# lyndonchan/wsss-analysis

Hardware: AMD Instinct MI355X
Metric: images/sec CAM+CRF pseudo-labels, VOC2012 321x321 (higher is better)
Workload: dtype f16x3; 1 GPU; resnet50 CAM + dense-CRF (M=21, 10 mean-field iters), 321x321, batch 32 images (=64 samples) per GPU, image-sharded; batch_images=32, num_classes=20, parallelism=image-sharded x1, no collective, steps_per_rank=239

## Files before the change

### __graft_entry__.py

```python
import os
import subprocess
import sys

ROOT = os.path.dirname(os.path.abspath(__file__))
PKG_DIR = os.path.join(ROOT, "wsss-analysis_amd")
CSRC = os.path.join(PKG_DIR, "csrc")
LIB_OUT = os.path.join(PKG_DIR, "wsscam", "libwsscam.so")
ORACLE_DIR = os.path.join(ROOT, "oracle")
ORACLE_OUT = os.path.join(ORACLE_DIR, "_build", "libdensecrf_ref.so")

HIP_SOURCES = ["api.hip", "conv_igemm.hip", "misc_kernels.hip", "net.hip", "cam_tail.hip", "crf.hip", "irn_kernels.hip", "rw.hip", "hsn.hip", "input.hip", "ir_label.hip", "stem_pool.hip", "cam_head.hip", "conv_f32.hip", "dsrg.hip", "cue_seeds.hip", "seg_eval.hip", "deeplab.hip", "seg_chain.hip", "seg_loss.hip", "pool.hip", "seg_grad.hip", "seg_sgd.hip", "seg_dropout.hip", "irn_loss.hip", "irn_grad.hip", "irn_sgd.hip", "irn_batch.hip", "seg_batch.hip", "cls_head.hip", "cls_grad.hip", "cls_sgd.hip"]
EXTRA_FLAGS = {"crf.hip": ["-ffp-contract=off"], "input.hip": ["-ffp-contract=off"], "deeplab.hip": ["-ffp-contract=off"],
               "seg_chain.hip": ["-ffp-contract=off"],
               "seg_sgd.hip": ["-ffp-contract=off"],
               "seg_dropout.hip": ["-ffp-contract=off"],
               "irn_sgd.hip": ["-ffp-contract=off"],
               "irn_grad.hip": ["-ffp-contract=off"],
               "irn_batch.hip": ["-ffp-contract=off"],
               "cls_sgd.hip": ["-ffp-contract=off"],
               "seg_batch.hip": ["-ffp-contract=off"]}


def _newer(target, deps):
    if not os.path.exists(target):
        return False
    t = os.path.getmtime(target)
    return all(os.path.getmtime(d) <= t for d in deps)


def _run(cmd):
    r = subprocess.run(cmd, stdout=subprocess.PIPE, stderr=subprocess.STDOUT, text=True)
    if r.returncode != 0:
        raise RuntimeError("command failed: %s\n%s" % (" ".join(cmd), r.stdout))
    return r.stdout


def build_lib(force=False, verbose=False):
    hipcc = os.environ.get("HIPCC", "/opt/rocm/bin/hipcc")
    objdir = os.path.join(PKG_DIR, "build")
    os.makedirs(objdir, exist_ok=True)
    os.makedirs(os.path.dirname(LIB_OUT), exist_ok=True)
    headers = [os.path.join(CSRC, "common.h"), os.path.join(CSRC, "bilerp.h"), os.path.join(CSRC, "tf_resize.h"),
               os.path.join(ROOT, "include", "wsscam.h")]
    if not force and _newer(LIB_OUT, [os.path.join(CSRC, src) for src in HIP_SOURCES] + headers):
        return LIB_OUT
    objs = []
    procs = []
    for src in HIP_SOURCES:
        sp = os.path.join(CSRC, src)
        op = os.path.join(objdir, src.replace(".hip", ".o"))
        objs.append(op)
        if not force and _newer(op, [sp] + headers):
            continue
        cmd = [hipcc, "--offload-arch=gfx950", "-O3", "-std=c++17", "-fPIC", "-Wall", "-c", sp, "-o", op] + EXTRA_FLAGS.get(src, [])
        if verbose:
            print(" ".join(cmd))
        procs.append((cmd, subprocess.Popen(cmd, stdout=subprocess.PIPE, stderr=subprocess.STDOUT, text=True)))
    for cmd, p in procs:
        out, _ = p.communicate()
        if p.returncode != 0:
            raise RuntimeError("hipcc failed: %s\n%s" % (" ".join(cmd), out))
        if verbose and out.strip():
            print(out)
    if force or procs or not _newer(LIB_OUT, objs):
        _run([hipcc, "--offload-arch=gfx950", "-shared", "-fPIC", "-o", LIB_OUT] + objs)
# ... 36 lines not shown
```

### include/wsscam.h

```cpp
#ifndef WSSCAM_H
#define WSSCAM_H

#include <stddef.h>
#include <stdint.h>

#ifdef __cplusplus
extern "C" {
#endif

#define WSC_VERSION 100

typedef enum wsc_status {
    WSC_OK = 0,
    WSC_ERR_INVALID = -1,
    WSC_ERR_NO_DEVICE = -2,
    WSC_ERR_HIP = -3,
    WSC_ERR_MISSING_KEY = -4,
    WSC_ERR_SHAPE = -5,
    WSC_ERR_NOMEM = -6,
    WSC_ERR_KEY_RANGE = -7,
    WSC_ERR_CAPACITY = -8,
    WSC_ERR_RANGE = -9
} wsc_status;

// ... 9 lines not shown
} wsc_arch;

typedef enum wsc_precision {
    WSC_PREC_BF16 = 0,
    WSC_PREC_BF16X3 = 1,
    WSC_PREC_F16 = 2,
    WSC_PREC_F16X3 = 3,
    WSC_PREC_F32 = 4
} wsc_precision;

typedef struct wsc_ctx wsc_ctx;
typedef struct wsc_net wsc_net;
typedef enum {
    WSC_OPT_CRF_GAUSS_ON_CHIP = 0,
    WSC_OPT_CRF_FUSED_BLUR = 1,
    WSC_OPT_CRF_BLUR_ON_CHIP = 2,
    WSC_OPT_CRF_RANK_BALLOT = 3,
    WSC_OPT_CRF_EMBED_FULL = 4,
    WSC_OPT_RW_TILED = 5,
    WSC_OPT_STEM_POOL_FUSED = 6,
    WSC_OPT_CONV_WINDOW = 7,
    WSC_OPT_CAM_HEAD_STREAM = 8,
    WSC_OPT_CRF_MSG_IN_UPDATE = 9,
    WSC_OPT_COUNT = 10
} wsc_option;

typedef struct wsc_crf wsc_crf;
typedef struct wsc_crf_v wsc_crf_v;

typedef struct wsc_tensor_desc {
    const char *name;
    const float *data;
    int32_t ndim;
    int64_t shape[4];
} wsc_tensor_desc;


int wsc_version(void);
const char *wsc_last_error(void);

int wsc_ctx_create(int device, void *stream, wsc_ctx **out);
void wsc_ctx_destroy(wsc_ctx *ctx);
int wsc_ctx_set_option(wsc_ctx *ctx, int option, int value);
int wsc_ctx_scratch_fill(wsc_ctx *ctx, int value);
int wsc_ctx_scratch_fill_value(const wsc_ctx *ctx);
int wsc_sync(wsc_ctx *ctx);
int wsc_ctx_range_status(wsc_ctx *ctx, int *flag_out, int clear);
// ... 401 lines not shown
```

### profiles/conv_layer_table.py

```python
import re
import sqlite3
import sys


def resnet50_layers(S):
    def o(h, k, s, p):
        return (h + 2 * p - k) // s + 1

    L = []
    h = o(S, 7, 2, 3)
    L.append(("stem 7x7 s2 3->64", h, 3, 64, 7))
    h = o(h, 3, 2, 1)
    inp = 64
    for li, (planes, blocks, stride) in enumerate(((64, 3, 1), (128, 4, 2), (256, 6, 2), (512, 3, 1)), 1):
        for b in range(blocks):
            s = stride if b == 0 else 1
            ho = o(h, 3, s, 1)
            n = "layer%d.%d." % (li, b)
            L.append((n + "conv1 1x1 %d->%d" % (inp, planes), h, inp, planes, 1))
            L.append((n + "conv2 3x3 %d s%d" % (planes, s), ho, planes, planes, 3))
            if b == 0:
                L.append((n + "conv3+proj 1x1 (%d+%d)->%d" % (planes, inp, planes * 4), ho, planes + inp, planes * 4, 1))
            else:
                L.append((n + "conv3 1x1 %d->%d +res" % (planes, planes * 4), ho, planes, planes * 4, 1))
# ... 2 lines not shown
    L.append(("CAM head 1x1 2048->20", h, 2048, 20, 1))
    return L


def n_dispatches(M, cin, cout, k, num_cus=256, planes=1):
    if cin % 64 or cout % 256:
        return 1
    nk = k * k * cin // (32 if planes == 2 else 64)
    blocks_sq = ((M + 255) // 256) * (cout // 256)
    if nk < (16 if planes == 2 else 4) or blocks_sq < 192:
        return 1
    rounds, rem = divmod(blocks_sq, num_cus)
    return 2 if rounds >= 1 and 0 < rem and rem * 2 <= num_cus else 1


def main(db, N=64, S=321, planes=1):
    c = sqlite3.connect(db)
    tabs = [r[0] for r in c.execute("select name from sqlite_master where type='table'")]
    kd = [t for t in tabs if "kernel_dispatch" in t][0]
    ks = [t for t in tabs if "kernel_symbol" in t][0]
    rows = c.execute("select s.kernel_name, d.start, d.end, d.grid_size_x / d.workgroup_size_x, d.group_segment_size "
                     "from %s d join %s s on d.kernel_id = s.id order by d.start" % (kd, ks)).fetchall()
    start = [i for i, r in enumerate(rows) if "nchw_to_nhwc4" in r[0]][-1]
    convs = [r for r in rows[start:] if "conv_igemm_kernel" in r[0] or "stem_pool_kernel" in r[0] or "cam_head_kernel" in r[0]]
    layers = resnet50_layers(S)
    if "stem_pool_kernel" in convs[0][0]:
        layers[0] = ("stem 7x7 s2 3->64 + maxpool (fused)",) + layers[0][1:]
    print("%-44s %8s %8s %9s %7s %6s" % ("layer", "us", "TFLOP/s", "act TB/s", "blocks", "LDS KB"))
    tot = 0.0
    pos = 0
    for (name, ho, cin, cout, k) in layers:
        M = N * ho * ho
        nd = n_dispatches(M, cin, cout, k, planes=planes)
        rs = convs[pos:pos + nd]
        pos += nd
        us = sum(r[2] - r[1] for r in rs) / 1000.0
        tot += us
        fl = 2.0 * M * cout * k * k * cin
        by = 2.0 * M * cout * (2 if "+res" in name else 1) + 2.0 * N * (ho * (2 if "s2" in name else 1)) ** 2 * cin
        if "fused" in name:
            by = 8.0 * N * S * S + 2.0 * N * ((ho + 1) // 2) ** 2 * cout
        by *= planes
        print("%-44s %8.1f %8.0f %9.2f %7s %6s" % (name, us, fl / us / 1e6, by / us / 1e6, "+".join(str(r[3]) for r in rs),
                                                    "/".join("%.0f" % (r[4] / 1024.0) for r in rs)))
    print("conv kernels total %.1f us" % tot)


if __name__ == "__main__":
    main(sys.argv[1], *(int(v) for v in sys.argv[2:]))
```

### wsss-analysis_amd/csrc/api.hip

```cpp
#include "common.h"

#include <cerrno>
#include <cstdarg>
#include <fcntl.h>
#include <mutex>
#include <set>
#include <sys/uio.h>
#include <unistd.h>
#include <vector>
#include <cstdio>
#include <cstring>

static thread_local char g_err[1024] = "";

void wsc_set_error(const char *fmt, ...) {
    va_list ap;
    va_start(ap, fmt);
    vsnprintf(g_err, sizeof(g_err), fmt, ap);
    va_end(ap);
}

int wsc_set_max_dynamic_lds(wsc_ctx *ctx, const void *fn, int bytes) {
    static std::mutex mu;
    static std::set<std::pair<const void *, int>> done;
// ... 121 lines not shown
    (void)hipEventCreate(&e);
    return e;
}

WscKernelTimer::WscKernelTimer(wsc_ctx *c, int cls, double work) : ctx(c) {
    if (!ctx->profiling) return;
    WscProfRecord r;
    r.cls = cls;
    r.work = work;
    r.e0 = prof_event(ctx);
    r.e1 = prof_event(ctx);
    (void)hipEventRecord(r.e0, ctx->stream);
    ctx->prof.push_back(r);
    idx = (int)ctx->prof.size() - 1;
}
WscKernelTimer::~WscKernelTimer() {
    if (idx >= 0) (void)hipEventRecord(ctx->prof[idx].e1, ctx->stream);
}

static const char *kClassNames[WSC_K_COUNT] = {
    "conv_igemm_kernel<256-row tiles,glds>", "conv_igemm_kernel<128x128,glds>", "conv_igemm_kernel<128x64,glds>", "conv_igemm_kernel<small-Cin> / stem_pool_kernel",
    "pool/layout/flip-add", "cam_tail+unary", "crf_build(all)", "gauss_msg_kernel", "combine4+blur_lds+blur4+blur3_tile",
    "update_splat_kernel", "crf init/finish", "wgrad_kernel+reduce", "grad mask/bias/pool", "relu_up_grad_kernel",
    "gn_grad partial+columns+finish+apply"};

int wsc_ctx_range_check(wsc_ctx *ctx) {
    const unsigned f = *(volatile unsigned *)ctx->range_host;
    if (f == 0u) return WSC_OK;
    wsc_set_error("an activation of an IEEE-half conv mode (f16 / f16x3) reached half's ceiling (|v| >= 65504) in a layer with %u "
                  "output channels and was saturated -- the reference's fp32 would have kept it, these maps are not the reference's: "
                  "a model that saturates runs in WSC_PREC_F32, the exact fp32 mode.  Or a tensor of %u channels given to a network, a "
                  "layer or a parameter load held NaN / inf: no precision helps then, the input or the parameters are wrong "
                  "(wsc_ctx_range_status clears the flag)", f, f);
    return WSC_ERR_RANGE;
}

extern "C" {

int wsc_profile_begin(wsc_ctx *ctx) {
    WSC_CHECK(ctx, WSC_ERR_INVALID, "wsc_profile_begin: null ctx");
    WSC_HIP(hipStreamSynchronize(ctx->stream));
    for (auto &r : ctx->prof) {
        ctx->prof_pool.push_back(r.e0);
        ctx->prof_pool.push_back(r.e1);
    }
    ctx->prof.clear();
    ctx->profiling = true;
// ... 321 lines not shown
```

### wsss-analysis_amd/csrc/common.h

```cpp
#pragma once
#include <hip/hip_runtime.h>
#include <assert.h>
#include <stdint.h>
#include <map>
#include <string>
#include <unordered_map>
#include <vector>

#include "../../include/wsscam.h"

typedef uint16_t bf16_t;

typedef __bf16 bf16x8_t __attribute__((ext_vector_type(8)));
typedef _Float16 f16x8_t __attribute__((ext_vector_type(8)));
typedef float f32x16_t __attribute__((ext_vector_type(16)));
typedef float f32x4_t __attribute__((ext_vector_type(4)));

__host__ __device__ inline bf16_t f32_to_bf16(float f) {
    union { float f; uint32_t u; } v;
    v.f = f;
    uint32_t u = v.u;
    if ((u & 0x7fffffffu) > 0x7f800000u) return (bf16_t)((u >> 16) | 0x40);
    u += 0x7fffu + ((u >> 16) & 1u);
    return (bf16_t)(u >> 16);
// ... 71 lines not shown
    } while (0)
#define WSC_TRY(expr)                                                                          \
    do {                                                                                       \
        int _s = (expr);                                                                       \
        if (_s != WSC_OK) return _s;                                                           \
    } while (0)

enum WscKernelClass {
    WSC_K_CONV256 = 0,
    WSC_K_CONV128,
    WSC_K_CONV64,
    WSC_K_CONV_SMALLCIN,
    WSC_K_POOL_MISC,
    WSC_K_CAM_TAIL,
    WSC_K_CRF_BUILD,
    WSC_K_GAUSS_MSG,
    WSC_K_BLUR,
    WSC_K_SLICE_UPDATE,
    WSC_K_CRF_MISC,
    WSC_K_WGRAD,
    WSC_K_GRAD_MISC,
    WSC_K_UPSAMPLE_GRAD,
    WSC_K_GN_GRAD,
    WSC_K_COUNT
};
struct WscProfRecord {
    int cls;
    double work;
    hipEvent_t e0, e1;
};

struct WscGaussCache;
void wsc_gauss_cache_destroy(WscGaussCache *cache);
struct wsc_ctx {
    int device = 0;
    hipStream_t stream = nullptr;
    bool own_stream = false;
    int num_cus = 0;
    std::string arch;
    void *ws = nullptr;
    size_t ws_bytes = 0;
    static constexpr int PIN_SLOTS = 8;
    struct PinSlot {
        void *p = nullptr;
        size_t bytes = 0;
        hipEvent_t ev = nullptr;
        bool busy = false;
    };
    PinSlot pin_ring[PIN_SLOTS];
    int pin_next = 0;
    int opt[WSC_OPT_COUNT] = {1, 1, 1, 0, 0, -1, 1, 1, 1, 1};
    void *zero_page = nullptr;
    unsigned *range_host = nullptr, *range_dev = nullptr;
    hipEvent_t ev0 = nullptr, ev1 = nullptr;
    hipEvent_t join_ev = nullptr;
    hipEvent_t marks[8] = {};
    bool mark_set[8] = {};
    hipStream_t aux_stream = nullptr;
    hipEvent_t fork_ev = nullptr, aux_done_ev = nullptr;
    bool profiling = false;
    std::vector<WscProfRecord> prof;
    std::vector<hipEvent_t> prof_pool;
    std::multimap<size_t, void *> free_blocks;
    std::unordered_map<void *, size_t> live_blocks;
    WscGaussCache *gauss_cache = nullptr;
    int scratch_fill = -1;
};
int wsc_ctx_workspace(wsc_ctx *ctx, size_t bytes, void **out);
int wsc_ctx_range_check(wsc_ctx *ctx);
__device__ __forceinline__ unsigned half2_at_ceiling(unsigned hw) { return (hw & 0x7fff7fffu) + 0x04010401u; }
struct WscKernelTimer {
    wsc_ctx *ctx;
    int idx = -1;
    WscKernelTimer(wsc_ctx *c, int cls, double work);
// ... 173 lines not shown
    const void *w;
    const float *s1, *b1;
    const float *s2, *b2;
    Act res;
    Act y;
    float *y_f32;
    int N, H, W, Cin, Ho, Wo, Cout, CoutPad;
    int kh, kw, stride, pad;
    int dil = 1;
    int relu;
    ConvForm form;
    wsc_precision prec;
    int generic;
    int ldy;
    Act x2;
    int H2, W2, C2, stride2;
    bool operands_match() const {
        for (const Act *a : {&x, &res, &y, &x2})
            if (*a && a->prec != prec) return false;
        return true;
    }
};
int conv_igemm_launch(wsc_ctx *ctx, const ConvLaunch &p);
int conv_f32_launch(wsc_ctx *ctx, const ConvLaunch &p);
int launch_cam_head(wsc_ctx *ctx, Act x, int M, int K, const bf16_t *w, int Kw, int CoutPad, const float *s1, const float *b1,
                    int C, int relu, float *y);

inline int wsc_grid_for(long long total, int block = 256, int cap = 256 * 16) {
    long long g = (total + block - 1) / block;
    if (g > cap) g = cap;
    if (g < 1) g = 1;
    return (int)g;
}
inline unsigned *layer_door(wsc_ctx *ctx, wsc_precision prec) { return conv_fmt(prec) == 1 ? ctx->range_dev : nullptr; }
int launch_nchw_to_nhwc4(wsc_ctx *ctx, const float *x, int N, int H, int W, Act y, unsigned *range);
void stem_pool_input_dims(int H, int W, int *Hp, int *Wp);
int launch_stem_pool(wsc_ctx *ctx, Act x, int N, int H, int W, const bf16_t *w, int Kw, const float *s1, const float *b1, int relu,
                     Act y);
int launch_gather_strided(wsc_ctx *ctx, Act x, int N, int H, int W, int C, int stride, int Ho, int Wo, Act y, int ldy);
int launch_nchw_to_nhwc4_pad(wsc_ctx *ctx, const float *x, int N, int H, int W, int Hp, int Wp, int pad, Act y, unsigned *range);
int launch_flip_add(wsc_ctx *ctx, const float *head, int B, int h, int w, int C, int Cs, float *cam);
int launch_gap_linear_sigmoid(wsc_ctx *ctx, Act feat, int B, int hw, int F, const float *Wc, const float *bias, int C, float *score,
                              int sample_stride);
int launch_act_to_f32(wsc_ctx *ctx, Act x, size_t n, float *y);
int launch_nchw_to_nhwc(wsc_ctx *ctx, const float *x, int N, int C, int HW, Act y, unsigned *range);
int launch_nhwc_to_nchw(wsc_ctx *ctx, Act x, int N, int C, int HW, float *y);
// ... 149 lines not shown
```

### wsss-analysis_amd/csrc/conv_igemm.hip

```cpp
#include "common.h"

#include <type_traits>

namespace {

constexpr int BK = 64;

struct ConvKArgs {
    const bf16_t *x, *x_lo, *w;
    const float *s1, *b1, *s2, *b2;
    const bf16_t *res, *res_lo;
    bf16_t *y, *y_lo;
    float *y_f32;
    int H, W, Cin, Ho, Wo, Cout;
    int ldy;
    int kh, kw, stride, pad, relu;
    int M, HoWo;
    int m_base, m_end;
    unsigned div_howo_mul, div_howo_s1, div_howo_s2, div_wo_mul, div_wo_s1, div_wo_s2;
    int cchunks;
    int dil;
    int ksteps_base;
    int nk;
    int Kw;
    int Kbase;
    int ntiles_n, nblocks;
    const bf16_t *zero;
    int spare1;
    long long lo_delta;
    const bf16_t *x2;
    long long lo_delta2;
    int cc2, H2, W2, C2, stride2;
    int ldx;
    int win_npix;
    int spare2, spare3;
    unsigned *range;
};

__device__ __forceinline__ int lds_off(int row, int slot) {
    return row * 128 + ((slot ^ ((row >> 1) & 7)) << 4);
}

__device__ __forceinline__ void decode_row(const ConvKArgs &p, int m, int &n, int &ho, int &wo) {
    const unsigned t1 = __umulhi(p.div_howo_mul, (unsigned)m);
    n = (int)((t1 + (((unsigned)m - t1) >> p.div_howo_s1)) >> p.div_howo_s2);
    const int rem = m - n * p.HoWo;
    const unsigned t2 = __umulhi(p.div_wo_mul, (unsigned)rem);
    ho = (int)((t2 + (((unsigned)rem - t2) >> p.div_wo_s1)) >> p.div_wo_s2);
    wo = rem - ho * p.Wo;
}

template <int BM, int BN, int MODE, int SPLIT, int ET, int STAGES, int FAST = 0, int WPT = 0>
__global__ __launch_bounds__(BM * 2, (STAGES == 1 && FAST != 0) ? 4 : 2) void conv_igemm_kernel(ConvKArgs p) {
    constexpr bool GLDS = MODE == 0;
    constexpr int WMT = BM == 256 ? 128 : 64;
    constexpr bool FEPI = (FAST & 1) != 0, PW = (FAST & 2) != 0;
    constexpr bool WIN = WPT > 0;
    static_assert(!WIN || (SPLIT == 2 && BM == 128 && STAGES == 2 && FAST == 1), "LDS window: single-staged split, 128-row tile");
    static_assert(FAST == 0 || (SPLIT != 1 && ET == 1 && (MODE == 0 || FAST == 1)),
                  "FAST paths: f16, one plane or the single-staged split; the pointwise prologue belongs to the LDS-DMA layers");
    static_assert(SPLIT != 2 || (MODE == 0 && STAGES == 2), "single-staged split: LDS-DMA layers, two LDS buffers");
    static_assert(STAGES == 2 || SPLIT == 0, "one LDS buffer serves a one-K-step layer, which a layer of three K segments never is");
    constexpr int CK = SPLIT == 2 ? 32 : 64;
    constexpr int NT = BM * 2;
// ... 907 lines not shown
```

### wsss-analysis_amd/csrc/net.hip

```cpp
#include "common.h"

#include <algorithm>
#include <cmath>
#include <cstring>
#include <unordered_map>

namespace {

struct HostTensor {
    const float *data;
    int ndim;
    int64_t shape[4];
    int64_t numel() const {
        int64_t n = 1;
        for (int i = 0; i < ndim; ++i) n *= shape[i];
        return n;
    }
};
typedef std::unordered_map<std::string, HostTensor> Dict;

struct ConvW {
    void *w = nullptr;
    float *s1 = nullptr, *b1 = nullptr, *s2 = nullptr, *b2 = nullptr;
    int Cin = 0, Cout = 0, CoutPad = 0, kh = 1, kw = 1, stride = 1, pad = 0, relu = 0;
// ... 791 lines not shown
        in_pad = c0.pad;
        fused_stem = stem_pool_fused(ctx, net);
        if (fused_stem) {
            stem_pool_input_dims(S, SW, &in_h, &in_w);
            in_pad = 5;
        }
    }
    const size_t in_elems = (size_t)N * in_h * in_w * 4;
    void *ws;
    WSC_TRY(wsc_ctx_workspace(ctx, act_bytes(in_elems, net->prec) + 4 * act_bytes(pl.max_act, net->prec) + align_up(extra_bytes, 256), &ws));
    char *p = (char *)ws;
    const Act xin = act_carve(p, in_elems, net->prec);
    Act buf[4];
    for (Act &b : buf) b = act_carve(p, pl.max_act, net->prec);
    if (taps)
        for (int op : net->taps) taps->push_back(act_carve(p, pl.out_elems(N, op), net->prec));
    *extra = (void *)p;

    if (nhwc_in) {
        WSC_CHECK(in_pad == 0, WSC_ERR_INVALID, "internal: an NHWC input has no padded-stem form");
        WSC_TRY(launch_nhwc3_to_nhwc4(ctx, x_dev, N, S, SW, xin));
    } else if (in_pad > 0) WSC_TRY(launch_nchw_to_nhwc4_pad(ctx, x_dev, N, S, SW, in_h, in_w, in_pad, xin, ctx->range_dev));
    else WSC_TRY(launch_nchw_to_nhwc4(ctx, x_dev, N, S, SW, xin, ctx->range_dev));
    for (size_t i = 0; i < net->ops.size(); ++i) {
        const Op &op = net->ops[i];
        const OpDims &d = pl.ops[i];
        const Act src = op.in < 0 ? xin : buf[op.in];
        if (fused_stem && i == 0) continue;
        if (fused_stem && i == 1) {
            const ConvW &c0 = net->convs[net->ops[0].conv];
            WSC_TRY(launch_stem_pool(ctx, xin, N, S, SW, (const bf16_t *)c0.w, conv_k_layout(c0.kh, c0.kw, c0.Cin, c0.form, net->prec).Kw, c0.s1,
                                     c0.b1, c0.relu, buf[op.out]));
        } else if (op.type == OP_CONV) {
            const ConvW &c = net->convs[op.conv];
            ConvLaunch L = conv_launch(c, net->prec);
            L.x = src;
            if (op.res >= 0) L.res = buf[op.res];
            L.y = buf[op.out].at(op.coff);
            L.ldy = op.pitch;
            if (op.in2 >= 0) {
                L.x2 = buf[op.in2];
                L.H2 = d.H2; L.W2 = d.W2; L.C2 = d.C2; L.stride2 = op.ps;
            }
            L.N = N; L.H = d.H; L.W = d.W; L.Ho = d.Ho; L.Wo = d.Wo;
            if (c.form == CONV_FORM_STEM_ROWS && op.in < 0) on_padded_input(L, in_h, in_w);
            if (bn_train) L.s2 = L.b2 = nullptr;
            WSC_TRY(conv_igemm_launch(ctx, L));
        } else if (op.type == OP_GATHER) {
            WSC_TRY(launch_gather_strided(ctx, src, N, d.H, d.W, d.C, op.ps, d.Ho, d.Wo, buf[op.out].at(op.coff), op.pitch));
        } else {
            PoolGeom g;
            WSC_CHECK(pool_geom(op.rule, op.pk, op.ps, op.pp, op.avg, d.H, d.W, &g), WSC_ERR_INVALID, "internal: a pool plan_dims let through");
            WSC_TRY(launch_pool(ctx, src, N, d.H, d.W, d.C, g, buf[op.out]));
        }
        if (trace && trace->off[i] >= 0) WSC_TRY(launch_act_to_f32(ctx, buf[op.out], pl.out_elems(N, (int)i), trace->out + trace->off[i]));
        if (bn_train && op.type == OP_CONV && net->convs[op.conv].bn >= 0)
            WSC_TRY(bn_train_step(ctx, net, *bn_train, (int)i, (long long)N * d.Ho * d.Wo, buf[op.out]));
        if (taps)
            for (size_t k = 0; k < net->taps.size(); ++k)
                if (net->taps[k] == (int)i) {
                    const size_t nb = pl.out_elems(N, (int)i) * conv_elem_bytes(net->prec);
                    WSC_HIP(hipMemcpyAsync((*taps)[k].hi, buf[op.out].hi, nb, hipMemcpyDeviceToDevice, ctx->stream));
                    if (buf[op.out].lo) WSC_HIP(hipMemcpyAsync((*taps)[k].lo, buf[op.out].lo, nb, hipMemcpyDeviceToDevice, ctx->stream));
                }
    }
    *feat = buf[net->final_buf];
    if (xin_out) *xin_out = xin;
    if (spare) *spare = buf[net->final_buf == 3 ? 2 : 3];
    *hf = pl.hf;
    *wf = pl.wf;
    return WSC_OK;
}

int run_classifier(wsc_ctx *ctx, const wsc_net *net, Act feat, Act spare, int N, int count, int sample_stride, int hf, int wf,
                   float *score_dev) {
    int hw = hf * wf;
    if (net->cls_max && net->cls_pool_set) {
        const PoolSpec &ps = net->cls_pool;
        PoolGeom g;
        WSC_CHECK(pool_geom(ps.rule(), ps.k, ps.stride, 0, false, hf, wf, &g), WSC_ERR_INVALID,
                  "the %d x %d feature map is smaller than the classifier branch's %d x %d VALID pool", hf, wf, ps.k, ps.k);
        const bool crops = !ps.same && ((g.Ho - 1) * ps.stride + ps.k < hf || (g.Wo - 1) * ps.stride + ps.k < wf);
        if (crops) {
            WSC_TRY(launch_pool(ctx, feat, N, hf, wf, net->F, g, spare));
            feat = spare;
            hw = g.Ho * g.Wo;
        }
// ... 1795 lines not shown
```

### wsss-analysis_amd/wsscam/_lib.py

```python
import ctypes
import os
import re
import threading

import numpy as np

_HERE = os.path.dirname(os.path.abspath(__file__))
LIB_PATH = os.path.join(_HERE, "libwsscam.so")
HEADER_PATH = os.path.normpath(os.path.join(_HERE, "..", "..", "include", "wsscam.h"))

WSC_OK = 0
WSC_ERR_INVALID = -1
WSC_ERR_NO_DEVICE = -2
WSC_ERR_HIP = -3
WSC_ERR_MISSING_KEY = -4
WSC_ERR_SHAPE = -5
WSC_ERR_NOMEM = -6
WSC_ERR_KEY_RANGE = -7
WSC_ERR_CAPACITY = -8
WSC_ERR_RANGE = -9

ARCH_RESNET50_CAM = 0
ARCH_VGG16_CAM = 1
ARCH_M7_CAM = 2
ARCH_RESNET50_IRN = 3
ARCH_VGG16_IRN = 4
ARCH_M7_IRN = 5
ARCH_DEEPLAB_LFOV = 6
ARCH_DEEPLAB_ASPP = 7

PREC_BF16 = 0
PREC_BF16X3 = 1
PREC_F16 = 2
PREC_F16X3 = 3
PREC_F32 = 4
OPT_CRF_GAUSS_ON_CHIP, OPT_CRF_FUSED_BLUR, OPT_CRF_BLUR_ON_CHIP, OPT_CRF_RANK_BALLOT, OPT_CRF_EMBED_FULL, OPT_RW_TILED, \
    OPT_STEM_POOL_FUSED, OPT_CONV_WINDOW, OPT_CAM_HEAD_STREAM, OPT_CRF_MSG_IN_UPDATE = range(10)
OPT_DEFAULTS = {OPT_CRF_GAUSS_ON_CHIP: 1, OPT_CRF_FUSED_BLUR: 1, OPT_CRF_BLUR_ON_CHIP: 1, OPT_CRF_RANK_BALLOT: 0,
                OPT_CRF_EMBED_FULL: 0, OPT_RW_TILED: -1, OPT_STEM_POOL_FUSED: 1, OPT_CONV_WINDOW: 1, OPT_CAM_HEAD_STREAM: 1,
                OPT_CRF_MSG_IN_UPDATE: 1}
CONV_GENERIC = 0x100


class WscError(RuntimeError):
    def __init__(self, status, message):
        super().__init__("libwsscam error %d: %s" % (status, message))
        self.status = status


class TensorDesc(ctypes.Structure):
    _fields_ = [
        ("name", ctypes.c_char_p),
        ("data", ctypes.POINTER(ctypes.c_float)),
        ("ndim", ctypes.c_int32),
        ("shape", ctypes.c_int64 * 4),
    ]


class TraceOp(ctypes.Structure):
    _fields_ = [(n, ctypes.c_int32) for n in (
        "kind", "in_", "in2", "res", "Ho", "Wo", "C", "coff", "pitch", "kh", "kw", "stride", "pad", "dil", "relu", "affine2", "stride2",
        "pool_rule", "pool_k", "pool_stride", "pool_pad", "pool_avg", "fused_next")] + [("label", ctypes.c_char * 100)]

# ... 1519 lines not shown
```

Baseline: 2619 images/s.

## Fuse ResNet bottleneck conv3+residual with next block's conv1 in one chain kernel

Adds a conv_chain_kernel that computes a 1x1 conv3 (64->256) with its residual add and the following block's 1x1 conv1 (256->64) in one persistent kernel. The conv3 output tile is staged in LDS and fed straight into the second GEMM, so the second layer never re-reads the 256-channel activation from global memory and one launch is saved. The kernel is enabled by default for f16x3 and swaps activation buffers to place the second output. It only applies to layer1-shaped (64/256 channel) pairs, and the fixed 64-row tile with one block per CU may give lower MFMA utilisation than the tuned igemm kernels.

```diff
diff --git a/__graft_entry__.py b/__graft_entry__.py
--- a/__graft_entry__.py
+++ b/__graft_entry__.py
@@ -9,7 +9,7 @@
 ORACLE_DIR = os.path.join(ROOT, "oracle")
 ORACLE_OUT = os.path.join(ORACLE_DIR, "_build", "libdensecrf_ref.so")
 
-HIP_SOURCES = ["api.hip", "conv_igemm.hip", "misc_kernels.hip", "net.hip", "cam_tail.hip", "crf.hip", "irn_kernels.hip", "rw.hip", "hsn.hip", "input.hip", "ir_label.hip", "stem_pool.hip", "cam_head.hip", "conv_f32.hip", "dsrg.hip", "cue_seeds.hip", "seg_eval.hip", "deeplab.hip", "seg_chain.hip", "seg_loss.hip", "pool.hip", "seg_grad.hip", "seg_sgd.hip", "seg_dropout.hip", "irn_loss.hip", "irn_grad.hip", "irn_sgd.hip", "irn_batch.hip", "seg_batch.hip", "cls_head.hip", "cls_grad.hip", "cls_sgd.hip"]
+HIP_SOURCES = ["api.hip", "conv_igemm.hip", "misc_kernels.hip", "net.hip", "cam_tail.hip", "crf.hip", "irn_kernels.hip", "rw.hip", "hsn.hip", "input.hip", "ir_label.hip", "stem_pool.hip", "cam_head.hip", "conv_f32.hip", "dsrg.hip", "cue_seeds.hip", "seg_eval.hip", "deeplab.hip", "seg_chain.hip", "seg_loss.hip", "pool.hip", "seg_grad.hip", "seg_sgd.hip", "seg_dropout.hip", "irn_loss.hip", "irn_grad.hip", "irn_sgd.hip", "irn_batch.hip", "seg_batch.hip", "cls_head.hip", "cls_grad.hip", "cls_sgd.hip", "conv_chain.hip"]
 EXTRA_FLAGS = {"crf.hip": ["-ffp-contract=off"], "input.hip": ["-ffp-contract=off"], "deeplab.hip": ["-ffp-contract=off"],
                "seg_chain.hip": ["-ffp-contract=off"],
                "seg_sgd.hip": ["-ffp-contract=off"],
@@ -40,7 +40,7 @@
     objdir = os.path.join(PKG_DIR, "build")
     os.makedirs(objdir, exist_ok=True)
     os.makedirs(os.path.dirname(LIB_OUT), exist_ok=True)
-    headers = [os.path.join(CSRC, "common.h"), os.path.join(CSRC, "bilerp.h"), os.path.join(CSRC, "tf_resize.h"),
+    headers = [os.path.join(CSRC, "common.h"), os.path.join(CSRC, "bilerp.h"), os.path.join(CSRC, "tf_resize.h"), os.path.join(CSRC, "conv_tile.h"),
                os.path.join(ROOT, "include", "wsscam.h")]
     if not force and _newer(LIB_OUT, [os.path.join(CSRC, src) for src in HIP_SOURCES] + headers):
         return LIB_OUT
diff --git a/include/wsscam.h b/include/wsscam.h
--- a/include/wsscam.h
+++ b/include/wsscam.h
@@ -55,7 +55,8 @@
     WSC_OPT_CONV_WINDOW = 7,
     WSC_OPT_CAM_HEAD_STREAM = 8,
     WSC_OPT_CRF_MSG_IN_UPDATE = 9,
-    WSC_OPT_COUNT = 10
+    WSC_OPT_CONV_CHAIN = 10,
+    WSC_OPT_COUNT = 11
 } wsc_option;
 
 typedef struct wsc_crf wsc_crf;
diff --git a/profiles/conv_layer_table.py b/profiles/conv_layer_table.py
--- a/profiles/conv_layer_table.py
+++ b/profiles/conv_layer_table.py
@@ -48,15 +48,31 @@
     rows = c.execute("select s.kernel_name, d.start, d.end, d.grid_size_x / d.workgroup_size_x, d.group_segment_size "
                      "from %s d join %s s on d.kernel_id = s.id order by d.start" % (kd, ks)).fetchall()
     start = [i for i, r in enumerate(rows) if "nchw_to_nhwc4" in r[0]][-1]
-    convs = [r for r in rows[start:] if "conv_igemm_kernel" in r[0] or "stem_pool_kernel" in r[0] or "cam_head_kernel" in r[0]]
+    convs = [r for r in rows[start:] if "conv_igemm_kernel" in r[0] or "stem_pool_kernel" in r[0] or "cam_head_kernel" in r[0] or "conv_chain_kernel" in r[0]]
     layers = resnet50_layers(S)
     if "stem_pool_kernel" in convs[0][0]:
         layers[0] = ("stem 7x7 s2 3->64 + maxpool (fused)",) + layers[0][1:]
     print("%-44s %8s %8s %9s %7s %6s" % ("layer", "us", "TFLOP/s", "act TB/s", "blocks", "LDS KB"))
     tot = 0.0
     pos = 0
-    for (name, ho, cin, cout, k) in layers:
+    skip = False
+    for li, (name, ho, cin, cout, k) in enumerate(layers):
+        if skip:
+            skip = False
+            continue
         M = N * ho * ho
+        if pos < len(convs) and "conv_chain_kernel" in convs[pos][0]:
+            r = convs[pos]
+            pos += 1
+            skip = True
+            n2, _, cin2, cout2, _ = layers[li + 1]
+            us = (r[2] - r[1]) / 1000.0
+            tot += us
+            fl = 2.0 * M * (cout * cin + cout2 * cin2)
+            by = planes * 2.0 * M * (cin + 2 * cout + cout2)
+            print("%-44s %8.1f %8.0f %9.2f %7s %6s" % ("  chained: " + name.split(" ")[0] + " -> " + n2.split(" ")[0], us, fl / us / 1e6,
+                                                        by / us / 1e6, str(r[3]), "%.0f" % (r[4] / 1024.0)))
+            continue
         nd = n_dispatches(M, cin, cout, k, planes=planes)
         rs = convs[pos:pos + nd]
         pos += nd
diff --git a/wsss-analysis_amd/csrc/api.hip b/wsss-analysis_amd/csrc/api.hip
--- a/wsss-analysis_amd/csrc/api.hip
+++ b/wsss-analysis_amd/csrc/api.hip
@@ -167,7 +167,7 @@
     "conv_igemm_kernel<256-row tiles,glds>", "conv_igemm_kernel<128x128,glds>", "conv_igemm_kernel<128x64,glds>", "conv_igemm_kernel<small-Cin> / stem_pool_kernel",
     "pool/layout/flip-add", "cam_tail+unary", "crf_build(all)", "gauss_msg_kernel", "combine4+blur_lds+blur4+blur3_tile",
     "update_splat_kernel", "crf init/finish", "wgrad_kernel+reduce", "grad mask/bias/pool", "relu_up_grad_kernel",
-    "gn_grad partial+columns+finish+apply"};
+    "gn_grad partial+columns+finish+apply", "conv_igemm_kernel pair as conv_chain_kernel<conv3+res -> conv1>"};
 
 int wsc_ctx_range_check(wsc_ctx *ctx) {
     const unsigned f = *(volatile unsigned *)ctx->range_host;
diff --git a/wsss-analysis_amd/csrc/common.h b/wsss-analysis_amd/csrc/common.h
--- a/wsss-analysis_amd/csrc/common.h
+++ b/wsss-analysis_amd/csrc/common.h
@@ -117,6 +117,7 @@
     WSC_K_GRAD_MISC,
     WSC_K_UPSAMPLE_GRAD,
     WSC_K_GN_GRAD,
+    WSC_K_CONV_CHAIN,
     WSC_K_COUNT
 };
 struct WscProfRecord {
@@ -144,7 +145,7 @@
     };
     PinSlot pin_ring[PIN_SLOTS];
     int pin_next = 0;
-    int opt[WSC_OPT_COUNT] = {1, 1, 1, 0, 0, -1, 1, 1, 1, 1};
+    int opt[WSC_OPT_COUNT] = {1, 1, 1, 0, 0, -1, 1, 1, 1, 1, 1};
     void *zero_page = nullptr;
     unsigned *range_host = nullptr, *range_dev = nullptr;
     hipEvent_t ev0 = nullptr, ev1 = nullptr;
@@ -364,6 +365,8 @@
     }
 };
 int conv_igemm_launch(wsc_ctx *ctx, const ConvLaunch &p);
+bool conv_chain_takes(const wsc_ctx *ctx, const ConvLaunch &c3, const ConvLaunch &c1);
+int conv_chain_launch(wsc_ctx *ctx, const ConvLaunch &c3, const ConvLaunch &c1);
 int conv_f32_launch(wsc_ctx *ctx, const ConvLaunch &p);
 int launch_cam_head(wsc_ctx *ctx, Act x, int M, int K, const bf16_t *w, int Kw, int CoutPad, const float *s1, const float *b1,
                     int C, int relu, float *y);
diff --git a/wsss-analysis_amd/csrc/conv_chain.hip b/wsss-analysis_amd/csrc/conv_chain.hip
--- /dev/null
+++ b/wsss-analysis_amd/csrc/conv_chain.hip
@@ -0,0 +1,325 @@
+#include "common.h"
+#include "conv_tile.h"
+
+namespace {
+
+constexpr int CH_TM = 64;
+constexpr int CH_K1 = 64, CH_N1 = 256;
+constexpr int CH_N2 = 64;
+constexpr int CH_CHUNK = CH_TM * 128;
+constexpr int CH_A_BYTES = (CH_K1 / 32) * CH_CHUNK;
+constexpr int CH_A2_BYTES = (CH_N1 / 32) * CH_CHUNK;
+constexpr int CH_W1_BYTES = (CH_N1 / 32) * CH_N2 * 128;
+constexpr int CH_LDS = CH_A_BYTES + CH_A2_BYTES + CH_W1_BYTES;
+static_assert(CH_LDS < 160 * 1024, "LDS budget of a CU");
+static_assert(4 * 32 * 32 * 4 <= CH_A_BYTES, "the per-wave fp32 transposes fit the dead A tile");
+
+struct ChainArgs {
+    const bf16_t *a;
+    long long a_lo_delta;
+    const bf16_t *w3;
+    const float *s3, *b3;
+    const bf16_t *res, *res_lo;
+    bf16_t *y1, *y1_lo;
+    const bf16_t *w1;
+    const float *s1, *b1;
+    bf16_t *y2, *y2_lo;
+    int M, ntiles;
+    unsigned *range;
+};
+
+typedef unsigned u32x4_t __attribute__((ext_vector_type(4)));
+
+__device__ __forceinline__ f32x16_t mfma_f16(const u32x4_t &a, const u32x4_t &b, const f32x16_t &c) {
+    return __builtin_amdgcn_mfma_f32_32x32x16_f16(__builtin_bit_cast(f16x8_t, a), __builtin_bit_cast(f16x8_t, b), c, 0, 0, 0);
+}
+__device__ __forceinline__ void lds_fence() { asm volatile("s_waitcnt lgkmcnt(0)" ::: "memory"); }
+__device__ __forceinline__ void lds_barrier() {
+    lds_fence();
+    __builtin_amdgcn_s_barrier();
+    asm volatile("" ::: "memory");
+}
+__device__ __forceinline__ int ct_row(int row) { return row ^ ((row >> 2) & 1); }
+
+template <bool RES>
+__device__ __forceinline__ void chain_epilogue8(const f32x4_t &q0, const f32x4_t &q1, const float (&s)[8], const float (&b)[8],
+                                                const u32x4_t &rh, const u32x4_t &rl, uint32_t (&hw)[4], uint32_t (&lw)[4]) {
+    float v[8];
+#pragma unroll
+    for (int j = 0; j < 4; ++j) {
+        v[j] = q0[j] * s[j] + b[j];
+        v[4 + j] = q1[j] * s[4 + j] + b[4 + j];
+    }
+    if (RES) {
+#pragma unroll
+        for (int j = 0; j < 4; ++j) {
+            v[2 * j] += f16_to_f32((bf16_t)(rh[j] & 0xffffu));
+            v[2 * j + 1] += f16_to_f32((bf16_t)(rh[j] >> 16));
+        }
+#pragma unroll
+        for (int j = 0; j < 4; ++j) {
+            v[2 * j] += f16_to_f32((bf16_t)(rl[j] & 0xffffu));
+            v[2 * j + 1] += f16_to_f32((bf16_t)(rl[j] >> 16));
+        }
+    }
+#pragma unroll
+    for (int j = 0; j < 4; ++j) {
+        const float c0 = __builtin_amdgcn_fmed3f(v[2 * j], 0.f, 65504.f), c1 = __builtin_amdgcn_fmed3f(v[2 * j + 1], 0.f, 65504.f);
+        const _Float16 h0 = (_Float16)c0;
+        const _Float16 h1 = (_Float16)c1;
+        hw[j] = (uint32_t)__builtin_bit_cast(uint16_t, h0) | ((uint32_t)__builtin_bit_cast(uint16_t, h1) << 16);
+        const _Float16 l0 = (_Float16)(c0 - (float)h0), l1 = (_Float16)(c1 - (float)h1);
+        lw[j] = (uint32_t)__builtin_bit_cast(uint16_t, l0) | ((uint32_t)__builtin_bit_cast(uint16_t, l1) << 16);
+    }
+}
+
+__global__ __launch_bounds__(256, 1) void conv_chain_kernel(ChainArgs p) {
+    extern __shared__ __attribute__((aligned(16))) char smem[];
+    char *const sA = smem, *const sA2 = smem + CH_A_BYTES, *const sW1 = smem + CH_A_BYTES + CH_A2_BYTES;
+
+    const int t = threadIdx.x;
+    const int lane = t & 63;
+    const int wv = __builtin_amdgcn_readfirstlane(t >> 6);
+    const int l31 = lane & 31, kgrp = lane >> 5;
+    const int c4 = lane & 3, r16 = lane >> 2;
+    const int wm = wv >> 1, wn = wv & 1;
+    float *const ct = reinterpret_cast<float *>(sA + wv * 4096);
+
+    for (int g = t; g < (CH_N1 / 32) * CH_N2 * 8; g += 256) {
+        const int kc = g >> 9, row = (g >> 3) & 63, slot = g & 7;
+        *reinterpret_cast<u32x4_t *>(sW1 + kc * (CH_N2 * 128) + lds_off(row, slot)) =
+            *reinterpret_cast<const u32x4_t *>(p.w1 + row * (CH_N1 * 2) + kc * 64 + slot * 8);
+    }
+    u32x4_t w3h[2][2][2], w3l[2][2][2];
+#pragma unroll
+    for (int ni = 0; ni < 2; ++ni)
+#pragma unroll
+        for (int c = 0; c < 2; ++c)
+#pragma unroll
+            for (int sl = 0; sl < 2; ++sl) {
+                const bf16_t *w = p.w3 + (wv * 64 + ni * 32 + l31) * (CH_K1 * 2) + c * 64 + (sl * 2 + kgrp) * 8;
+                w3h[ni][c][sl] = *reinterpret_cast<const u32x4_t *>(w);
+                w3l[ni][c][sl] = *reinterpret_cast<const u32x4_t *>(w + 32);
+            }
+    float s3[2][8], b3[2][8], s1[8], b1[8];
+#pragma unroll
+    for (int ni = 0; ni < 2; ++ni) {
+        const int c = wv * 64 + ni * 32 + c4 * 8;
+        const f32x4_t sa = *reinterpret_cast<const f32x4_t *>(p.s3 + c), sb = *reinterpret_cast<const f32x4_t *>(p.s3 + c + 4);
+        const f32x4_t ba = *reinterpret_cast<const f32x4_t *>(p.b3 + c), bb = *reinterpret_cast<const f32x4_t *>(p.b3 + c + 4);
+#pragma unroll
+        for (int j = 0; j < 4; ++j) {
+            s3[ni][j] = sa[j]; s3[ni][4 + j] = sb[j]; b3[ni][j] = ba[j]; b3[ni][4 + j] = bb[j];
+        }
+    }
+    {
+        const int c = wn * 32 + c4 * 8;
+        const f32x4_t sa = *reinterpret_cast<const f32x4_t *>(p.s1 + c), sb = *reinterpret_cast<const f32x4_t *>(p.s1 + c + 4);
+        const f32x4_t ba = *reinterpret_cast<const f32x4_t *>(p.b1 + c), bb = *reinterpret_cast<const f32x4_t *>(p.b1 + c + 4);
+#pragma unroll
+        for (int j = 0; j < 4; ++j) {
+            s1[j] = sa[j]; s1[4 + j] = sb[j]; b1[j] = ba[j]; b1[4 + j] = bb[j];
+        }
+    }
+
+    struct Rows {
+        u32x4_t a[4], h[2][2][2], l[2][2][2];
+    };
+    auto request = [&](int tile, Rows &r) __attribute__((always_inline)) {
+        const int m0 = tile * CH_TM;
+#pragma unroll
+        for (int j = 0; j < 4; ++j) {
+            const int g = j * 256 + t, row = g >> 4, s = g & 15;
+            const int m = m0 + row < p.M ? m0 + row : p.M - 1;
+            r.a[j] = *reinterpret_cast<const u32x4_t *>(p.a + (((s & 8) ? p.a_lo_delta : 0ll) + (long long)((unsigned)m * (unsigned)CH_K1 + (unsigned)((s & 7) * 8))));
+        }
+#pragma unroll
+        for (int mi = 0; mi < 2; ++mi)
+#pragma unroll
+            for (int pass = 0; pass < 2; ++pass) {
+                const int row = m0 + mi * 32 + pass * 16 + r16;
+                const int m = row < p.M ? row : p.M - 1;
+#pragma unroll
+                for (int ni = 0; ni < 2; ++ni) {
+                    const unsigned o = (unsigned)m * (unsigned)CH_N1 + (unsigned)(wv * 64 + ni * 32 + c4 * 8);
+                    r.h[mi][ni][pass] = *reinterpret_cast<const u32x4_t *>(p.res + o);
+                    r.l[mi][ni][pass] = *reinterpret_cast<const u32x4_t *>(p.res_lo + o);
+                }
+            }
+    };
+
+#pragma unroll
+    for (int ni = 0; ni < 2; ++ni)
+#pragma unroll
+        for (int c = 0; c < 2; ++c)
+#pragma unroll
+            for (int sl = 0; sl < 2; ++sl) asm volatile("" : "+v"(w3h[ni][c][sl]), "+v"(w3l[ni][c][sl]));
+#pragma unroll
+    for (int j = 0; j < 8; ++j) asm volatile("" : "+v"(s3[0][j]), "+v"(s3[1][j]), "+v"(b3[0][j]), "+v"(b3[1][j]), "+v"(s1[j]), "+v"(b1[j]));
+    unsigned ovf2 = 0u;
+    auto one_tile = [&](int tile, Rows &cur, Rows &nxt) __attribute__((always_inline)) {
+        const int m0 = tile * CH_TM;
+#pragma unroll
+        for (int j = 0; j < 4; ++j) {
+            const int g = j * 256 + t, row = g >> 4, s = g & 15;
+            *reinterpret_cast<u32x4_t *>(sA + ((s & 7) >> 2) * CH_CHUNK + lds_off(row, (s & 3) + ((s & 8) ? 4 : 0))) = cur.a[j];
+        }
+        if (tile + (int)gridDim.x < p.ntiles) request(tile + (int)gridDim.x, nxt);
+        lds_barrier();
+
+        f32x16_t acc[2][2];
+#pragma unroll
+        for (int mi = 0; mi < 2; ++mi)
+#pragma unroll
+            for (int ni = 0; ni < 2; ++ni)
+#pragma unroll
+                for (int r = 0; r < 16; ++r) acc[mi][ni][r] = 0.f;
+#pragma unroll
+        for (int c = 0; c < 2; ++c)
+#pragma unroll
+            for (int sl = 0; sl < 2; ++sl) {
+                u32x4_t ah[2], al[2];
+#pragma unroll
+                for (int mi = 0; mi < 2; ++mi) {
+                    ah[mi] = *reinterpret_cast<const u32x4_t *>(sA + c * CH_CHUNK + lds_off(mi * 32 + l31, sl * 2 + kgrp));
+                    al[mi] = *reinterpret_cast<const u32x4_t *>(sA + c * CH_CHUNK + lds_off(mi * 32 + l31, 4 + sl * 2 + kgrp));
+                }
+#pragma unroll
+                for (int mi = 0; mi < 2; ++mi)
+#pragma unroll
+                    for (int ni = 0; ni < 2; ++ni) acc[mi][ni] = mfma_f16(al[mi], w3h[ni][c][sl], acc[mi][ni]);
+#pragma unroll
+                for (int mi = 0; mi < 2; ++mi)
+#pragma unroll
+                    for (int ni = 0; ni < 2; ++ni) acc[mi][ni] = mfma_f16(ah[mi], w3l[ni][c][sl], acc[mi][ni]);
+#pragma unroll
+                for (int mi = 0; mi < 2; ++mi)
+#pragma unroll
+                    for (int ni = 0; ni < 2; ++ni) acc[mi][ni] = mfma_f16(ah[mi], w3h[ni][c][sl], acc[mi][ni]);
+            }
+        lds_barrier();
+
+        unsigned ovf1 = 0u;
+#pragma unroll
+        for (int mi = 0; mi < 2; ++mi) {
+#pragma unroll
+            for (int ni = 0; ni < 2; ++ni) {
+                const int c = wv * 64 + ni * 32 + c4 * 8;
+                lds_fence();
+#pragma unroll
+                for (int r = 0; r < 16; ++r) ct[ct_row((r & 3) + 8 * (r >> 2) + 4 * kgrp) * 32 + l31] = acc[mi][ni][r];
+                lds_fence();
+#pragma unroll
+                for (int pass = 0; pass < 2; ++pass) {
+                    const int rr = pass * 16 + r16;
+                    const f32x4_t q0 = *reinterpret_cast<const f32x4_t *>(ct + ct_row(rr) * 32 + c4 * 8);
+                    const f32x4_t q1 = *reinterpret_cast<const f32x4_t *>(ct + ct_row(rr) * 32 + c4 * 8 + 4);
+                    uint32_t hw[4], lw[4];
+                    chain_epilogue8<true>(q0, q1, s3[ni], b3[ni], cur.h[mi][ni][pass], cur.l[mi][ni][pass], hw, lw);
+                    const u32x4_t vh = {hw[0], hw[1], hw[2], hw[3]}, vl = {lw[0], lw[1], lw[2], lw[3]};
+                    const int row = mi * 32 + rr, m = m0 + row;
+                    if (m < p.M) {
+                        ovf1 |= half2_at_ceiling(hw[0]) | half2_at_ceiling(hw[1]) | half2_at_ceiling(hw[2]) | half2_at_ceiling(hw[3]);
+                        const unsigned o = (unsigned)m * (unsigned)CH_N1 + (unsigned)c;
+                        *reinterpret_cast<u32x4_t *>(p.y1 + o) = vh;
+                        *reinterpret_cast<u32x4_t *>(p.y1_lo + o) = vl;
+                    }
+                    char *const a2 = sA2 + (wv * 2 + ni) * CH_CHUNK;
+                    *reinterpret_cast<u32x4_t *>(a2 + lds_off(row, c4)) = vh;
+                    *reinterpret_cast<u32x4_t *>(a2 + lds_off(row, 4 + c4)) = vl;
+                }
+            }
+        }
+        if (ovf1 & 0x80008000u) *p.range = (unsigned)CH_N1;
+        lds_barrier();
+
+        f32x16_t acc2;
+#pragma unroll
+        for (int r = 0; r < 16; ++r) acc2[r] = 0.f;
+#pragma unroll
+        for (int kc = 0; kc < CH_N1 / 32; ++kc)
+#pragma unroll
+            for (int sl = 0; sl < 2; ++sl) {
+                const char *const a2 = sA2 + kc * CH_CHUNK, *const w = sW1 + kc * (CH_N2 * 128);
+                const u32x4_t ah = *reinterpret_cast<const u32x4_t *>(a2 + lds_off(wm * 32 + l31, sl * 2 + kgrp));
+                const u32x4_t al = *reinterpret_cast<const u32x4_t *>(a2 + lds_off(wm * 32 + l31, 4 + sl * 2 + kgrp));
+                const u32x4_t bh = *reinterpret_cast<const u32x4_t *>(w + lds_off(wn * 32 + l31, sl * 2 + kgrp));
+                const u32x4_t bl = *reinterpret_cast<const u32x4_t *>(w + lds_off(wn * 32 + l31, 4 + sl * 2 + kgrp));
+                acc2 = mfma_f16(al, bh, acc2);
+                acc2 = mfma_f16(ah, bl, acc2);
+                acc2 = mfma_f16(ah, bh, acc2);
+            }
+
+        lds_fence();
+#pragma unroll
+        for (int r = 0; r < 16; ++r) ct[ct_row((r & 3) + 8 * (r >> 2) + 4 * kgrp) * 32 + l31] = acc2[r];
+        lds_fence();
+#pragma unroll
+        for (int pass = 0; pass < 2; ++pass) {
+            const int rr = pass * 16 + r16;
+            const f32x4_t q0 = *reinterpret_cast<const f32x4_t *>(ct + ct_row(rr) * 32 + c4 * 8);
+            const f32x4_t q1 = *reinterpret_cast<const f32x4_t *>(ct + ct_row(rr) * 32 + c4 * 8 + 4);
+            uint32_t hw[4], lw[4];
+            const u32x4_t none = {0u, 0u, 0u, 0u};
+            chain_epilogue8<false>(q0, q1, s1, b1, none, none, hw, lw);
+            const int m = m0 + wm * 32 + rr;
+            if (m < p.M) {
+                ovf2 |= half2_at_ceiling(hw[0]) | half2_at_ceiling(hw[1]) | half2_at_ceiling(hw[2]) | half2_at_ceiling(hw[3]);
+                const unsigned o = (unsigned)m * (unsigned)CH_N2 + (unsigned)(wn * 32 + c4 * 8);
+                *reinterpret_cast<u32x4_t *>(p.y2 + o) = u32x4_t{hw[0], hw[1], hw[2], hw[3]};
+                *reinterpret_cast<u32x4_t *>(p.y2_lo + o) = u32x4_t{lw[0], lw[1], lw[2], lw[3]};
+            }
+        }
+        lds_barrier();
+    };
+    Rows r0, r1;
+    int tile = blockIdx.x;
+    request(tile, r0);
+    for (;;) {
+        one_tile(tile, r0, r1);
+        if ((tile += gridDim.x) >= p.ntiles) break;
+        one_tile(tile, r1, r0);
+        if ((tile += gridDim.x) >= p.ntiles) break;
+    }
+    if (ovf2 & 0x80008000u) *p.range = (unsigned)CH_N2;
+}
+
+bool is_pointwise(const ConvLaunch &c, int Cin, int Cout) {
+    return c.form == CONV_FORM_GENERIC && c.kh == 1 && c.kw == 1 && c.stride == 1 && c.pad == 0 && c.Cin == Cin && c.Cout == Cout &&
+           c.CoutPad == Cout && c.relu == 1 && c.s2 == nullptr && c.y_f32 == nullptr && !c.x2 && !c.generic && (c.ldy == 0 || c.ldy == Cout) &&
+           c.x && c.y && c.x.lo && c.y.lo;
+}
+
+}
+
+bool conv_chain_takes(const wsc_ctx *ctx, const ConvLaunch &c3, const ConvLaunch &c1) {
+    if (c3.prec != WSC_PREC_F16X3 || c1.prec != WSC_PREC_F16X3 || ctx->num_cus <= 0) return false;
+    if (!is_pointwise(c3, CH_K1, CH_N1) || !is_pointwise(c1, CH_N1, CH_N2)) return false;
+    if (!c3.res || !c3.res.lo || c1.res || !c3.operands_match() || !c1.operands_match()) return false;
+    if (c1.x.hi != c3.y.hi || c1.x.lo != c3.y.lo) return false;
+    if (c1.N != c3.N || c1.Ho != c3.Ho || c1.Wo != c3.Wo || c1.H != c3.Ho || c1.W != c3.Wo || c3.H != c3.Ho || c3.W != c3.Wo) return false;
+    for (const Act *a : {&c3.x, &c3.res, &c3.y})
+        if (a->hi == c1.y.hi) return false;
+    const long long M = (long long)c3.N * c3.Ho * c3.Wo;
+    return M > 0 && M * CH_N1 < (1ll << 31);
+}
+
+int conv_chain_launch(wsc_ctx *ctx, const ConvLaunch &c3, const ConvLaunch &c1) {
+    WSC_CHECK(conv_chain_takes(ctx, c3, c1), WSC_ERR_INVALID, "conv chain: not a 64 -> 256 (+ residual) -> 64 pair of f16x3 1x1 layers");
+    ChainArgs a = {};
+    a.a = c3.x.h16(); a.a_lo_delta = (long long)(c3.x.h16_lo() - c3.x.h16());
+    a.w3 = (const bf16_t *)c3.w; a.s3 = c3.s1; a.b3 = c3.b1;
+    a.res = c3.res.h16(); a.res_lo = c3.res.h16_lo();
+    a.y1 = c3.y.h16(); a.y1_lo = c3.y.h16_lo();
+    a.w1 = (const bf16_t *)c1.w; a.s1 = c1.s1; a.b1 = c1.b1;
+    a.y2 = c1.y.h16(); a.y2_lo = c1.y.h16_lo();
+    a.M = c3.N * c3.Ho * c3.Wo;
+    a.ntiles = (a.M + CH_TM - 1) / CH_TM;
+    a.range = ctx->range_dev;
+    WSC_TRY(wsc_set_max_dynamic_lds(ctx, reinterpret_cast<const void *>(conv_chain_kernel), CH_LDS));
+    const int grid = a.ntiles < ctx->num_cus ? a.ntiles : ctx->num_cus;
+    WscKernelTimer timer(ctx, WSC_K_CONV_CHAIN, 2.0 * a.M * ((double)CH_N1 * CH_K1 + (double)CH_N2 * CH_N1));
+    hipLaunchKernelGGL(conv_chain_kernel, dim3(grid), dim3(256), CH_LDS, ctx->stream, a);
+    WSC_HIP(hipGetLastError());
+    return WSC_OK;
+}
diff --git a/wsss-analysis_amd/csrc/conv_igemm.hip b/wsss-analysis_amd/csrc/conv_igemm.hip
--- a/wsss-analysis_amd/csrc/conv_igemm.hip
+++ b/wsss-analysis_amd/csrc/conv_igemm.hip
@@ -1,4 +1,5 @@
 #include "common.h"
+#include "conv_tile.h"
 
 #include <type_traits>
 
@@ -36,10 +37,6 @@
     int spare2, spare3;
     unsigned *range;
 };
-
-__device__ __forceinline__ int lds_off(int row, int slot) {
-    return row * 128 + ((slot ^ ((row >> 1) & 7)) << 4);
-}
 
 __device__ __forceinline__ void decode_row(const ConvKArgs &p, int m, int &n, int &ho, int &wo) {
     const unsigned t1 = __umulhi(p.div_howo_mul, (unsigned)m);
diff --git a/wsss-analysis_amd/csrc/conv_tile.h b/wsss-analysis_amd/csrc/conv_tile.h
--- /dev/null
+++ b/wsss-analysis_amd/csrc/conv_tile.h
@@ -0,0 +1,6 @@
+#pragma once
+#include "common.h"
+
+__device__ __forceinline__ int lds_off(int row, int slot) {
+    return row * 128 + ((slot ^ ((row >> 1) & 7)) << 4);
+}
diff --git a/wsss-analysis_amd/csrc/net.hip b/wsss-analysis_amd/csrc/net.hip
--- a/wsss-analysis_amd/csrc/net.hip
+++ b/wsss-analysis_amd/csrc/net.hip
@@ -837,6 +837,57 @@
         WSC_TRY(launch_nhwc3_to_nhwc4(ctx, x_dev, N, S, SW, xin));
     } else if (in_pad > 0) WSC_TRY(launch_nchw_to_nhwc4_pad(ctx, x_dev, N, S, SW, in_h, in_w, in_pad, xin, ctx->range_dev));
     else WSC_TRY(launch_nchw_to_nhwc4(ctx, x_dev, N, S, SW, xin, ctx->range_dev));
+    auto conv_op_launch = [&](size_t i) {
+        const Op &op = net->ops[i];
+        const OpDims &d = pl.ops[i];
+        const ConvW &c = net->convs[op.conv];
+        ConvLaunch L = conv_launch(c, net->prec);
+        L.x = op.in < 0 ? xin : buf[op.in];
+        if (op.res >= 0) L.res = buf[op.res];
+        L.y = buf[op.out].at(op.coff);
+        L.ldy = op.pitch;
+        if (op.in2 >= 0) {
+            L.x2 = buf[op.in2];
+            L.H2 = d.H2; L.W2 = d.W2; L.C2 = d.C2; L.stride2 = op.ps;
+        }
+        L.N = N; L.H = d.H; L.W = d.W; L.Ho = d.Ho; L.Wo = d.Wo;
+        if (c.form == CONV_FORM_STEM_ROWS && op.in < 0) on_padded_input(L, in_h, in_w);
+        if (bn_train) L.s2 = L.b2 = nullptr;
+        return L;
+    };
+    auto after_op = [&](size_t i) -> int {
+        const Op &op = net->ops[i];
+        const OpDims &d = pl.ops[i];
+        if (trace && trace->off[i] >= 0) WSC_TRY(launch_act_to_f32(ctx, buf[op.out], pl.out_elems(N, (int)i), trace->out + trace->off[i]));
+        if (bn_train && op.type == OP_CONV && net->convs[op.conv].bn >= 0)
+            WSC_TRY(bn_train_step(ctx, net, *bn_train, (int)i, (long long)N * d.Ho * d.Wo, buf[op.out]));
+        if (taps)
+            for (size_t k = 0; k < net->taps.size(); ++k)
+                if (net->taps[k] == (int)i) {
+                    const size_t nb = pl.out_elems(N, (int)i) * conv_elem_bytes(net->prec);
+                    WSC_HIP(hipMemcpyAsync((*taps)[k].hi, buf[op.out].hi, nb, hipMemcpyDeviceToDevice, ctx->stream));
+                    if (buf[op.out].lo) WSC_HIP(hipMemcpyAsync((*taps)[k].lo, buf[op.out].lo, nb, hipMemcpyDeviceToDevice, ctx->stream));
+                }
+        return WSC_OK;
+    };
+    auto chain_buffer = [&](size_t i) -> int {
+        if (!ctx->opt[WSC_OPT_CONV_CHAIN] || net->prec != WSC_PREC_F16X3 || bn_train || i + 1 >= net->ops.size()) return -1;
+        const Op &o3 = net->ops[i], &o1 = net->ops[i + 1];
+        if (o3.type != OP_CONV || o1.type != OP_CONV || o3.in < 0 || o3.res < 0 || o1.in != o3.out || o1.res >= 0 || o1.in2 >= 0) return -1;
+        int spare_id = -1;
+        for (int b = 0; b < 4; ++b)
+            if (b != o3.in && b != o3.res && b != o3.out) spare_id = b;
+        if (spare_id < 0 || spare_id == o1.out) return spare_id == o1.out ? o1.out : -1;
+        for (size_t j = i + 2; j < net->ops.size(); ++j) {
+            const Op &o = net->ops[j];
+            if (o.in == spare_id || o.res == spare_id || o.in2 == spare_id) return -1;
+            if (o.out == spare_id) {
+                if (o.pitch || o.type == OP_GATHER) return -1;
+                return spare_id;
+            }
+        }
+        return net->final_buf == spare_id ? -1 : spare_id;
+    };
     for (size_t i = 0; i < net->ops.size(); ++i) {
         const Op &op = net->ops[i];
         const OpDims &d = pl.ops[i];
@@ -847,20 +898,21 @@
             WSC_TRY(launch_stem_pool(ctx, xin, N, S, SW, (const bf16_t *)c0.w, conv_k_layout(c0.kh, c0.kw, c0.Cin, c0.form, net->prec).Kw, c0.s1,
                                      c0.b1, c0.relu, buf[op.out]));
         } else if (op.type == OP_CONV) {
-            const ConvW &c = net->convs[op.conv];
-            ConvLaunch L = conv_launch(c, net->prec);
-            L.x = src;
-            if (op.res >= 0) L.res = buf[op.res];
-            L.y = buf[op.out].at(op.coff);
-            L.ldy = op.pitch;
-            if (op.in2 >= 0) {
-                L.x2 = buf[op.in2];
-                L.H2 = d.H2; L.W2 = d.W2; L.C2 = d.C2; L.stride2 = op.ps;
+            const int cb = chain_buffer(i);
+            if (cb >= 0) {
+                const int o1 = net->ops[i + 1].out;
+                const ConvLaunch L3 = conv_op_launch(i);
+                std::swap(buf[cb], buf[o1]);
+                const ConvLaunch L1 = conv_op_launch(i + 1);
+                if (conv_chain_takes(ctx, L3, L1)) {
+                    WSC_TRY(conv_chain_launch(ctx, L3, L1));
+                    WSC_TRY(after_op(i));
+                    WSC_TRY(after_op(++i));
+                    continue;
+                }
+                std::swap(buf[cb], buf[o1]);
             }
-            L.N = N; L.H = d.H; L.W = d.W; L.Ho = d.Ho; L.Wo = d.Wo;
-            if (c.form == CONV_FORM_STEM_ROWS && op.in < 0) on_padded_input(L, in_h, in_w);
-            if (bn_train) L.s2 = L.b2 = nullptr;
-            WSC_TRY(conv_igemm_launch(ctx, L));
+            WSC_TRY(conv_igemm_launch(ctx, conv_op_launch(i)));
         } else if (op.type == OP_GATHER) {
             WSC_TRY(launch_gather_strided(ctx, src, N, d.H, d.W, d.C, op.ps, d.Ho, d.Wo, buf[op.out].at(op.coff), op.pitch));
         } else {
@@ -868,16 +920,7 @@
             WSC_CHECK(pool_geom(op.rule, op.pk, op.ps, op.pp, op.avg, d.H, d.W, &g), WSC_ERR_INVALID, "internal: a pool plan_dims let through");
             WSC_TRY(launch_pool(ctx, src, N, d.H, d.W, d.C, g, buf[op.out]));
         }
-        if (trace && trace->off[i] >= 0) WSC_TRY(launch_act_to_f32(ctx, buf[op.out], pl.out_elems(N, (int)i), trace->out + trace->off[i]));
-        if (bn_train && op.type == OP_CONV && net->convs[op.conv].bn >= 0)
-            WSC_TRY(bn_train_step(ctx, net, *bn_train, (int)i, (long long)N * d.Ho * d.Wo, buf[op.out]));
-        if (taps)
-            for (size_t k = 0; k < net->taps.size(); ++k)
-                if (net->taps[k] == (int)i) {
-                    const size_t nb = pl.out_elems(N, (int)i) * conv_elem_bytes(net->prec);
-                    WSC_HIP(hipMemcpyAsync((*taps)[k].hi, buf[op.out].hi, nb, hipMemcpyDeviceToDevice, ctx->stream));
-                    if (buf[op.out].lo) WSC_HIP(hipMemcpyAsync((*taps)[k].lo, buf[op.out].lo, nb, hipMemcpyDeviceToDevice, ctx->stream));
-                }
+        WSC_TRY(after_op(i));
     }
     *feat = buf[net->final_buf];
     if (xin_out) *xin_out = xin;
diff --git a/wsss-analysis_amd/wsscam/_lib.py b/wsss-analysis_amd/wsscam/_lib.py
--- a/wsss-analysis_amd/wsscam/_lib.py
+++ b/wsss-analysis_amd/wsscam/_lib.py
@@ -35,10 +35,10 @@
 PREC_F16X3 = 3
 PREC_F32 = 4
 OPT_CRF_GAUSS_ON_CHIP, OPT_CRF_FUSED_BLUR, OPT_CRF_BLUR_ON_CHIP, OPT_CRF_RANK_BALLOT, OPT_CRF_EMBED_FULL, OPT_RW_TILED, \
-    OPT_STEM_POOL_FUSED, OPT_CONV_WINDOW, OPT_CAM_HEAD_STREAM, OPT_CRF_MSG_IN_UPDATE = range(10)
+    OPT_STEM_POOL_FUSED, OPT_CONV_WINDOW, OPT_CAM_HEAD_STREAM, OPT_CRF_MSG_IN_UPDATE, OPT_CONV_CHAIN = range(11)
 OPT_DEFAULTS = {OPT_CRF_GAUSS_ON_CHIP: 1, OPT_CRF_FUSED_BLUR: 1, OPT_CRF_BLUR_ON_CHIP: 1, OPT_CRF_RANK_BALLOT: 0,
                 OPT_CRF_EMBED_FULL: 0, OPT_RW_TILED: -1, OPT_STEM_POOL_FUSED: 1, OPT_CONV_WINDOW: 1, OPT_CAM_HEAD_STREAM: 1,
-                OPT_CRF_MSG_IN_UPDATE: 1}
+                OPT_CRF_MSG_IN_UPDATE: 1, OPT_CONV_CHAIN: 1}
 CONV_GENERIC = 0x100
 
 
```

Result: no change. 2633 images/s, median of 2 (+0.5%).
